# decisiongraph/leann-rs

Hardware: AMD Instinct MI355X
Metric: queries/sec @ recall@10>=0.95 (higher is better)
Workload: dtype f32

## Files before the change

### leann-rs_amd/csrc/search.cuh

```cuda
#pragma once
#include "common.cuh"
#include "row_screen.h"
#include "search_plan.h"

struct GraphView {
    const float *X;
    const uint32_t *adj0;
    const uint32_t *adjU;
    const uint32_t *upper_off;
    uint64_t n;
    uint32_t d, ld, M, M0, max_level, entry;
    uint32_t feat_h, row_bytes;
    const float *norms;
};

#define GPOOL_TABLES 1024u
#define GPOOL_BITS 16u

struct SearchArgs {
    const float *queries;
    const uint32_t *q_rows;
    uint32_t ldq, nq, k, ef, target_level;
    uint32_t hash_bits;
    uint64_t key_offset;
    uint64_t *out_keys;
    float *out_dists;
    uint32_t *out_counts;
    uint32_t *out_stats;
    uint64_t *out_expanded;
    uint32_t *out_nexp;
    uint32_t exp_cap;
    unsigned long long *gpool;
    uint32_t *gpool_lock;
    uint32_t *gpool_ctr;
    uint32_t gpool_bits, gpool_tables;
    unsigned long long *gpool2;
    uint32_t *gpool2_lock;
    uint32_t gpool2_bits, gpool2_tables;
    const uint8_t *allow;
    uint64_t allow_stride;
    const uint16_t *x_hi, *x_lo;
    uint32_t ldp;
    unsigned long long *screen_ctr;
};

static_assert(alignof(SearchArgs) == 8 && alignof(GraphView) == 8, "lazy_search_args assumes `a` sits at the 8-byte aligned offset behind `g`");
__device__ __forceinline__ const __attribute__((address_space(4))) SearchArgs *lazy_search_args() {
    typedef const __attribute__((address_space(4))) char *kptr;
    return (const __attribute__((address_space(4))) SearchArgs *)((kptr)__builtin_amdgcn_kernarg_segment_ptr() +
                                                                  ((sizeof(GraphView) + 7) & ~(size_t)7));
}

__device__ __forceinline__ uint32_t uni(uint32_t v) { return (uint32_t)__builtin_amdgcn_readfirstlane((int)v); }

__device__ __forceinline__ uint32_t vis_hash(uint32_t id, uint32_t bits) {
    return (id * 0x9E3779B1u) >> (32 - bits);
}

__device__ __forceinline__ bool vis_insert_lds(uint32_t *tab, uint32_t bits, uint32_t id) {
    const uint32_t mask = (1u << bits) - 1u;
    uint32_t h = vis_hash(id, bits);
    for (;;) {
        uint32_t old = atomicCAS(&tab[h], LEANN_EMPTY, id);
        if (old == LEANN_EMPTY) return true;
        if (old == id) return false;
        h = (h + 1) & mask;
    }
}
__device__ __forceinline__ bool vis_insert_hbm(unsigned long long *tab, uint32_t bits, uint32_t gen, uint32_t id) {
    const uint32_t mask = (1u << bits) - 1u;
    uint32_t h = vis_hash(id, bits);
    const unsigned long long mine = ((unsigned long long)gen << 32) | id;
    for (;;) {
        unsigned long long cur = __hip_atomic_load(&tab[h], __ATOMIC_RELAXED, __HIP_MEMORY_SCOPE_AGENT);
        if ((uint32_t)(cur >> 32) != gen) {
            unsigned long long prev = atomicCAS(&tab[h], cur, mine);
            if (prev == cur) return true;
            continue;
        }
        if ((uint32_t)cur == id) return false;
        h = (h + 1) & mask;
    }
}

template <int T, int R>
__device__ __forceinline__ void wave_dist_rows(const float4 (&q)[T], const float *__restrict__ X, uint32_t ld,
                                               const uint32_t (&ids)[R], int nrows, int lane, float (&out)[R]) {
    float4 v[R][T];
#pragma unroll
    for (int r = 0; r < R; r++) {
        if (r < nrows) {
            const float *row = X + (size_t)ids[r] * ld;
#pragma unroll
            for (int t = 0; t < T; t++) v[r][t] = row_load4(row, ld, t, lane);
        }
    }
#pragma unroll
    for (int r = 0; r < R; r++) {
        if (r < nrows) {
            float4 acc = make_float4(0.f, 0.f, 0.f, 0.f);
#pragma unroll
            for (int t = 0; t < T; t++) fma4(acc, q[t], v[r][t]);
            out[r] = 1.0f - wave_tree_sum(lane4_sum(acc));
        }
    }
}

__device__ __forceinline__ uint2 plane_tail_load(const uint16_t *__restrict__ row, uint32_t ldp, int c, int lane) {
    const uint32_t j = 256u * c + 4u * lane;
    return j < ldp ? *reinterpret_cast<const uint2 *>(row + j) : make_uint2(0u, 0u);
}
template <int T>
__device__ __forceinline__ void plane_row_load(const uint16_t *__restrict__ row, uint32_t ldp, int lane, uint2 (&h)[T]) {
#pragma unroll
    for (int p = 0; p < T / 2; p++) {
        if (512u * (uint32_t)(p + 1) <= ldp) {
            const uint4 v = *reinterpret_cast<const uint4 *>(row + 512 * p + 8 * lane);
            h[2 * p] = make_uint2(v.x, v.y);
            h[2 * p + 1] = make_uint2(v.z, v.w);
        } else {
            h[2 * p] = plane_tail_load(row, ldp, 2 * p, lane);
            h[2 * p + 1] = plane_tail_load(row, ldp, 2 * p + 1, lane);
        }
    }
    if (T & 1) h[T - 1] = plane_tail_load(row, ldp, T - 1, lane);
}
template <int T, int R>
__device__ __forceinline__ uint32_t wave_dist_rows_screen(const float4 (&q)[T], const uint16_t *__restrict__ Xhi, const uint16_t *__restrict__ Xlo,
                                                          uint32_t ldp, const uint32_t (&ids)[R], int nrows, int lane, bool armed, float worst,
                                                          float E, float (&out)[R]) {
    uint2 h[R][T], l[R][T];
#pragma unroll
    for (int r = 0; r < R; r++)
        if (r < nrows) plane_row_load<T>(Xhi + (size_t)ids[r] * ldp, ldp, lane, h[r]);
    uint32_t ruled = 0;
#pragma unroll
    for (int r = 0; r < R; r++) {
        if (r < nrows) {
            float4 s = make_float4(0.f, 0.f, 0.f, 0.f), a = make_float4(0.f, 0.f, 0.f, 0.f);
#pragma unroll
            for (int t = 0; t < T; t++) {
                float4 x;
                x.x = __uint_as_float(h[r][t].x << 16);
                x.y = __uint_as_float(h[r][t].x & 0xFFFF0000u);
                x.z = __uint_as_float(h[r][t].y << 16);
                x.w = __uint_as_float(h[r][t].y & 0xFFFF0000u);
                fma4(s, q[t], x);
                a.x = fmaf(fabsf(q[t].x), fabsf(x.x), a.x);
                a.y = fmaf(fabsf(q[t].y), fabsf(x.y), a.y);
                a.z = fmaf(fabsf(q[t].z), fabsf(x.z), a.z);
                a.w = fmaf(fabsf(q[t].w), fabsf(x.w), a.w);
            }
            const float lb = rs_lower_bound(wave_tree_sum(rs_lane_bound(lane4_sum(s), lane4_sum(a))), E);
            out[r] = lb;
            if (armed && lb > worst) ruled |= 1u << r;
        }
    }
#pragma unroll
    for (int r = 0; r < R; r++)
        if (r < nrows && !((ruled >> r) & 1u)) plane_row_load<T>(Xlo + (size_t)ids[r] * ldp, ldp, lane, l[r]);
#pragma unroll
    for (int r = 0; r < R; r++) {
        if (r < nrows && !((ruled >> r) & 1u)) {
            float4 acc = make_float4(0.f, 0.f, 0.f, 0.f);
#pragma unroll
            for (int t = 0; t < T; t++) {
                float4 x;
                x.x = __uint_as_float((h[r][t].x << 16) | (l[r][t].x & 0xFFFFu));
                x.y = __uint_as_float((h[r][t].x & 0xFFFF0000u) | (l[r][t].x >> 16));
                x.z = __uint_as_float((h[r][t].y << 16) | (l[r][t].y & 0xFFFFu));
                x.w = __uint_as_float((h[r][t].y & 0xFFFF0000u) | (l[r][t].y >> 16));
                fma4(acc, q[t], x);
            }
            out[r] = 1.0f - wave_tree_sum(lane4_sum(acc));
        }
    }
    return ruled;
}

template <int T, int R>
__device__ __forceinline__ void wave_dist_rows_feat(const float4 (&q)[T], const char *__restrict__ Xb, uint32_t row_bytes,
                                                    uint32_t h, const uint32_t (&ids)[R], int nrows, int lane, float (&out)[R],
                                                    const float *__restrict__ norms = nullptr) {
    uint2 v[R][T];
    float nrm[R];
#pragma unroll
    for (int r = 0; r < R; r++) {
        if (r < nrows) {
            const char *row = Xb + (size_t)ids[r] * row_bytes;
#pragma unroll
            for (int t = 0; t < T; t++) {
                const uint32_t j = 256u * t + 4u * lane;
                v[r][t] = j < h ? *reinterpret_cast<const uint2 *>(row + 2 * (size_t)j) : make_uint2(0u, 0u);
            }
            nrm[r] = norms ? norms[ids[r]] : *reinterpret_cast<const float *>(row + 2 * (size_t)h);
        }
    }
#pragma unroll
    for (int r = 0; r < R; r++) {
        if (r < nrows) {
            float4 acc = make_float4(0.f, 0.f, 0.f, 0.f);
#pragma unroll
            for (int t = 0; t < T; t++) {
                float4 x;
                x.x = __uint_as_float(v[r][t].x << 16);
                x.y = __uint_as_float(v[r][t].x & 0xFFFF0000u);
                x.z = __uint_as_float(v[r][t].y << 16);
                x.w = __uint_as_float(v[r][t].y & 0xFFFF0000u);
                fma4(acc, q[t], x);
            }
            out[r] = 1.0f - wave_tree_sum(lane4_sum(acc)) / nrm[r];
        }
    }
}

template <int T, int R>
__device__ __forceinline__ void wave_dist_rows_bf16(const float4 (&q)[T], const uint16_t *__restrict__ Xb, uint32_t ldb,
                                                    const uint32_t (&ids)[R], int nrows, int lane, float (&out)[R]) {
    uint2 v[R][T];
#pragma unroll
    for (int r = 0; r < R; r++)
        if (r < nrows) plane_row_load<T>(Xb + (size_t)ids[r] * ldb, ldb, lane, v[r]);
#pragma unroll
    for (int r = 0; r < R; r++) {
        if (r < nrows) {
            float4 acc = make_float4(0.f, 0.f, 0.f, 0.f);
#pragma unroll
            for (int t = 0; t < T; t++) {
                float4 x;
                x.x = __uint_as_float(v[r][t].x << 16);
                x.y = __uint_as_float(v[r][t].x & 0xFFFF0000u);
                x.z = __uint_as_float(v[r][t].y << 16);
                x.w = __uint_as_float(v[r][t].y & 0xFFFF0000u);
                fma4(acc, q[t], x);
            }
            out[r] = 1.0f - wave_tree_sum(lane4_sum(acc));
        }
    }
}

typedef uint32_t u32x4_a8 __attribute__((ext_vector_type(4), aligned(8)));
__device__ __forceinline__ float feat8_partial_pair(const float (&q)[8], const u32x4_a8 v) {
    float4 lo, hi;
    lo.x = fmaf(q[0], __uint_as_float(v.x << 16), 0.f);
    lo.y = fmaf(q[1], __uint_as_float(v.x & 0xFFFF0000u), 0.f);
    lo.z = fmaf(q[2], __uint_as_float(v.y << 16), 0.f);
    lo.w = fmaf(q[3], __uint_as_float(v.y & 0xFFFF0000u), 0.f);
    hi.x = fmaf(q[4], __uint_as_float(v.z << 16), 0.f);
    hi.y = fmaf(q[5], __uint_as_float(v.z & 0xFFFF0000u), 0.f);
    hi.z = fmaf(q[6], __uint_as_float(v.w << 16), 0.f);
    hi.w = fmaf(q[7], __uint_as_float(v.w & 0xFFFF0000u), 0.f);
    return lane4_sum(lo) + lane4_sum(hi);
}
template <int G>
__device__ __forceinline__ void group_dist_rows_feat256(const float (&qa)[8], const float (&qb)[8], const char *__restrict__ Xb,
                                                        uint32_t row_bytes, const uint32_t (&id)[G], const bool (&valid)[G], int lane,
                                                        float (&out)[G], const float *__restrict__ norms) {
    const int m = lane & 15;
    u32x4_a8 va[G], vb[G];
    float nrm[G];
#pragma unroll
    for (int g = 0; g < G; g++) {
        va[g] = vb[g] = u32x4_a8{0u, 0u, 0u, 0u};
        nrm[g] = 1.f;
        if (valid[g]) {
            const char *row = Xb + (size_t)id[g] * row_bytes;
            va[g] = *reinterpret_cast<const u32x4_a8 *>(row + 16 * m);
            vb[g] = *reinterpret_cast<const u32x4_a8 *>(row + 256 + 16 * m);
            if (m == 15) nrm[g] = norms ? norms[id[g]] : *reinterpret_cast<const float *>(row + 512);
        }
    }
#pragma unroll
    for (int g = 0; g < G; g++) {
        float sa = feat8_partial_pair(qa, va[g]), sb = feat8_partial_pair(qb, vb[g]);
        sa = dpp_pair_add<0xB1, 0xf>(sa);
        sb = dpp_pair_add<0xB1, 0xf>(sb);
        sa = dpp_pair_add<0x4E, 0xf>(sa);
        sb = dpp_pair_add<0x4E, 0xf>(sb);
        sa = dpp_pair_add<0x114, 0xf>(sa);
        sb = dpp_pair_add<0x114, 0xf>(sb);
        sa = dpp_pair_add<0x118, 0xf>(sa);
        sb = dpp_pair_add<0x118, 0xf>(sb);
        out[g] = 1.0f - (sa + sb) / nrm[g];
    }
}

__device__ __forceinline__ const uint32_t *adj_list(const uint32_t *__restrict__ base, const uint32_t *__restrict__ upper_off, uint32_t deg,
                                                    int lv, uint32_t node) {
    const size_t list = lv == 0 ? (size_t)node : (size_t)upper_off[node] + (uint32_t)(lv - 1);
    return base + list * deg;
}

struct SearchLds {
    uint64_t *s_key;
    uint32_t *s_new;
    uint32_t *misc;
};

template <int T, int R, int NW, bool FEAT, bool FILT = false, bool G16 = false, int LW = 1, bool SCREEN = false, bool BF16 = false>
__device__ void beam_search_one(const GraphView &g, const SearchArgs &a, uint32_t qi, unsigned char *smem) {
    const int tid = threadIdx.x, lane = tid & 63, wave = tid >> 6;
    const auto *const za = lazy_search_args();
    const uint32_t ef = a.ef;
    static_assert(LW == 1 || LW == 2, "lists of at most 128 ids");
    static_assert(!SCREEN || (NW == 4 && !FEAT && !FILT && !G16 && LW == 1), "the row screen exists in the plain throughput form only");
    static_assert(!BF16 || (!FEAT && !G16 && !SCREEN), "bf16 rows: stored vectors, whole rows");
    const uint32_t maxdeg = g.M0 > g.M ? g.M0 : g.M;
    const uint32_t efp = (ef + 1) & ~1u;
    SearchLds s;
    uint64_t *const W0 = reinterpret_cast<uint64_t *>(smem);
    constexpr uint32_t NBUF = NW > 4 ? 2u : 1u;
    const uint32_t kstride = maxdeg + 8;
    s.s_key = W0 + 2 * efp;
    s.s_new = reinterpret_cast<uint32_t *>(s.s_key + NBUF * kstride);
    s.misc = s.s_new + NBUF * maxdeg;
    size_t off = 2 * (size_t)efp * 8 + NBUF * ((size_t)maxdeg + 8) * 8 + NBUF * (size_t)maxdeg * 4 + 64;
    off = (off + 15) & ~(size_t)15;
    const uint32_t kf = FILT ? a.k : 0u, kfp = (kf + 1) & ~1u;
    uint64_t *const R0 = reinterpret_cast<uint64_t *>(smem + off);
    uint64_t *const s_keyR = R0 + 2 * kfp;
    const uint8_t *const allow = FILT ? a.allow + (size_t)qi * a.allow_stride : nullptr;
    uint32_t rsize = 0;
    int rcur = 0;
    if (FILT) off += 2 * (size_t)kfp * 8 + NBUF * ((size_t)maxdeg + 8) * 8;
    uint32_t *table = reinterpret_cast<uint32_t *>(smem + off);
    const uint32_t hbits = a.hash_bits, hsize = 1u << hbits;
    uint32_t vis_limit = hsize - (hsize >> 2);
    uint32_t hbm = 0;
    unsigned long long *gtab = nullptr;
    uint32_t gslot = 0, gen = 0, gbits = 0;

    float4 q[T];
    float qa[8], qb[8];
    {
        const float *qv;
        uint32_t dq = FEAT ? g.feat_h : g.d;
        if (!FEAT && a.q_rows) qv = g.X + (size_t)a.q_rows[qi] * g.ld;
        else qv = a.queries + (size_t)qi * a.ldq;
#pragma unroll
        for (int t = 0; t < T; t++)
            if (!G16) q[t] = vec_load4_guard(qv, dq, t, lane);
        if (G16) {
#pragma unroll
            for (int i = 0; i < 8; i++) {
                qa[i] = qv[8 * (lane & 15) + i];
                qb[i] = qv[128 + 8 * (lane & 15) + i];
            }
        }
    }

    float rs_E = 0.f;
    uint32_t rs_ruled = 0;
    if constexpr (SCREEN) {
        float4 qs = make_float4(0.f, 0.f, 0.f, 0.f);
#pragma unroll
        for (int t = 0; t < T; t++) { qs.x += fabsf(q[t].x); qs.y += fabsf(q[t].y); qs.z += fabsf(q[t].z); qs.w += fabsf(q[t].w); }
        rs_E = rs_abs_term(wave_tree_sum(lane4_sum(qs)));
        if (tid == 0) s.misc[10] = 0;
    }
    const uint32_t *const adj0_p = g.adj0, *const adjU_p = g.adjU, *const upoff_p = g.upper_off;
    uint32_t n_evals = 1, hops0 = 0, hopsU = 0;
    uint32_t n_vis = 0;
    uint64_t best;
    {
        uint32_t ids[1] = {g.entry};
        float dd[1];
        if (G16) {
            const bool valid[1] = {lane < 16};
            group_dist_rows_feat256<1>(qa, qb, reinterpret_cast<const char *>(g.X), g.row_bytes, ids, valid, lane, dd, g.norms);
            dd[0] = __int_as_float(__builtin_amdgcn_readlane(__float_as_int(dd[0]), 15));
        } else if (FEAT) wave_dist_rows_feat<T, 1>(q, reinterpret_cast<const char *>(g.X), g.row_bytes, g.feat_h, ids, 1, lane, dd, g.norms);
        else if constexpr (BF16) wave_dist_rows_bf16<T, 1>(q, reinterpret_cast<const uint16_t *>(g.X), g.row_bytes >> 1, ids, 1, lane, dd);
        else wave_dist_rows<T, 1>(q, g.X, g.ld, ids, 1, lane, dd);
        best = make_key(dd[0], g.entry);
    }

#ifdef LEANN_STAMPS
    uint64_t stamp[8] = {0, 0, 0, 0, 0, 0, 0, 0};
#endif
    uint32_t wsize = 0, level_hops = 0;
    int cur = 0;
    bool aborted = false;
    for (int lv = (int)g.max_level; lv >= (int)a.target_level; --lv) {
        const uint32_t ef_l = (lv == (int)a.target_level) ? ef : 1u;
        const uint32_t deg = lv == 0 ? g.M0 : g.M;
        if (!hbm)
            for (uint32_t i = tid; i < hsize; i += NW * 64) table[i] = LEANN_EMPTY;
        __syncthreads();
        if (tid == 0) {
            W0[0] = best;
            if (hbm) {
                gen = atomicAdd(&za->gpool_ctr[1], 1u) + 1u;
                s.misc[5] = gen;
                vis_insert_hbm(gtab, gbits, gen, key_id(best));
            } else {
                table[vis_hash(key_id(best), hbits)] = key_id(best);
            }
            s.misc[1] = LEANN_EMPTY;
            s.misc[2] = LEANN_EMPTY;
            s.misc[3] = 0;
            if (FILT && lv == (int)a.target_level) {
                const uint32_t e = key_id(best);
                const uint32_t ok = (allow[e >> 3] >> (e & 7)) & 1u;
                if (ok) R0[0] = best;
                s.misc[6] = ok;
            }
        }
        __syncthreads();
        if (hbm) gen = uni(s.misc[5]);
        const bool filt_level = FILT && lv == (int)a.target_level;
        if (filt_level) { rsize = uni(s.misc[6]); rcur = 0; }
        cur = 0;
        wsize = 1;
        n_vis = 1;
        uint32_t sel = 0;
        uint32_t hop = 0;
        constexpr bool EARLY_B = NW > 4;
        if constexpr (!EARLY_B) {
            uint32_t e_pref = LEANN_EMPTY, e_pref1 = LEANN_EMPTY;
            const uint32_t *const adj_base = lv == 0 ? adj0_p : adjU_p;
            if (wave == 0) {
                e_pref = (uint32_t)lane < deg ? adj_list(adj_base, upoff_p, deg, lv, key_id(best))[lane] : LEANN_EMPTY;
                if constexpr (LW == 2) e_pref1 = (uint32_t)lane + 64u < deg ? adj_list(adj_base, upoff_p, deg, lv, key_id(best))[lane + 64] : LEANN_EMPTY;
            }
            while (sel != LEANN_EMPTY) {
                uint64_t *Wc = W0 + cur * efp, *Wn = W0 + (cur ^ 1) * efp;
    #ifdef LEANN_STAMPS
                const uint64_t st0 = __builtin_amdgcn_s_memtime();
    #endif
                if (wave == 0) {
                    constexpr uint32_t p = 0;
                    const uint64_t ckey = Wc[sel];
                    const uint32_t hidx = hop;
                    #include "hop_adj.cuh"
                }
    #ifdef LEANN_STAMPS
                const uint64_t stB = __builtin_amdgcn_s_memtime();
    #endif
                __syncthreads();
    #ifdef LEANN_STAMPS
                const uint64_t stB1 = __builtin_amdgcn_s_memtime();
    #endif
                const uint32_t table_full = uni(s.misc[3]);
                if (table_full) {
                    #include "hop_migrate.cuh"
                    continue;
                }
                const uint32_t n_new = uni(s.misc[0]);
                uint64_t *const skey = s.s_key, *const skeyR = s_keyR;
                const uint32_t *const snew = s.s_new;
                if constexpr (SCREEN) {
                    const bool armed = wsize == ef_l;
                    const float worst = orderable_f32(uni((uint32_t)(Wc[wsize - 1] >> 32)));
                    for (uint32_t j0 = wave; j0 < n_new; j0 += NW * R) {
                        uint32_t ids[R];
                        float dd[R];
                        int nrows = 0;
    #pragma unroll
                        for (int r = 0; r < R; r++) {
                            uint32_t j = j0 + r * NW;
                            if (j < n_new) { ids[r] = s.s_new[j]; nrows = r + 1; }
                        }
                        const uint32_t ruled = wave_dist_rows_screen<T, R>(q, za->x_hi, za->x_lo, za->ldp, ids, nrows, lane, armed, worst, rs_E, dd);
                        rs_ruled += (uint32_t)__popc(ruled);
                        if (lane == 0) {
    #pragma unroll
                            for (int r = 0; r < R; r++)
                                if (r < nrows) s.s_key[j0 + r * NW] = make_key(dd[r], ids[r]);
                        }
                    }
                } else {
                    #include "hop_rows.cuh"
                }
    #ifdef LEANN_STAMPS
                const uint64_t stC = __builtin_amdgcn_s_memtime();
    #endif
                __syncthreads();
    #ifdef LEANN_STAMPS
                const uint64_t stB2 = __builtin_amdgcn_s_memtime();
    #endif
                uint32_t *next_slot = &s.misc[1 + (hop & 1)];
                const uint32_t n_pad = (n_new + 7) & ~7u;
                if (wave == 0) {
                    #include "hop_select.cuh"
                } else {
                    #include "hop_merge.cuh"
                }
                if (filt_level) {
                    #include "hop_rmerge.cuh"
                }
    #ifdef LEANN_STAMPS
                const uint64_t stD = __builtin_amdgcn_s_memtime();
    #endif
                __syncthreads();
    #ifdef LEANN_STAMPS
                {
                    const uint64_t stE = __builtin_amdgcn_s_memtime();
                    stamp[0] += stB - st0; stamp[1] += stB1 - stB; stamp[2] += stC - stB1; stamp[3] += stB2 - stC;
                    stamp[4] += stD - stB2; stamp[5] += stE - stD; stamp[6] += 1;
                }
    #endif
                sel = uni(*next_slot);
                wsize = min(wsize + n_new, ef_l);
                cur ^= 1;
                hop++;
            }
        } else {
            const uint32_t *const adj_base = lv == 0 ? adj0_p : adjU_p;
            uint32_t e_pref = LEANN_EMPTY, e_pref1 = LEANN_EMPTY;
            auto phase_b = [&](uint32_t p, uint64_t ckey, uint32_t hidx) __attribute__((always_inline)) {
                #include "hop_adj.cuh"
            };
            if (wave == 0) {
                e_pref = (uint32_t)lane < deg ? adj_list(adj_base, upoff_p, deg, lv, key_id(best))[lane] : LEANN_EMPTY;
                if constexpr (LW == 2) e_pref1 = (uint32_t)lane + 64u < deg ? adj_list(adj_base, upoff_p, deg, lv, key_id(best))[lane + 64] : LEANN_EMPTY;
                phase_b(0u, best, 0u);
            }
            __syncthreads();
            uint32_t par = 0;
            for (;;) {
                uint64_t *Wc = W0 + cur * efp, *Wn = W0 + (cur ^ 1) * efp;
#ifdef LEANN_STAMPS
                const uint64_t st0 = __builtin_amdgcn_s_memtime();
#endif
                if (uni(s.misc[3])) {
                    #include "hop_migrate.cuh"
                    if (wave == 0) phase_b(par, Wc[sel], hop);
                    __syncthreads();
                    continue;
                }
                const uint32_t n_new = uni(s.misc[8 + par]);
                uint64_t *const skey = s.s_key + par * kstride;
                const uint32_t *const snew = s.s_new + par * maxdeg;
                uint64_t *const skeyR = s_keyR + par * kstride;
                #include "hop_rows.cuh"
#ifdef LEANN_STAMPS
                const uint64_t stC = __builtin_amdgcn_s_memtime();
#endif
                __syncthreads();
#ifdef LEANN_STAMPS
                const uint64_t stB2 = __builtin_amdgcn_s_memtime();
#endif
                uint32_t *next_slot = &s.misc[1 + (hop & 1)];
                const uint32_t n_pad = (n_new + 7) & ~7u;
                if (wave == 0) {
                    #include "hop_select.cuh"
                    if (next != LEANN_EMPTY) phase_b(par ^ 1u, ckey, hop + 1);
                } else {
                    #include "hop_merge.cuh"
                }
                if (filt_level) {
                    #include "hop_rmerge.cuh"
                }
#ifdef LEANN_STAMPS
                const uint64_t stD = __builtin_amdgcn_s_memtime();
#endif
                __syncthreads();
#ifdef LEANN_STAMPS
                {
                    const uint64_t stE = __builtin_amdgcn_s_memtime();
                    stamp[0] += 0; stamp[1] += 0; stamp[2] += stC - st0; stamp[3] += stB2 - stC;
                    stamp[4] += stD - stB2; stamp[5] += stE - stD; stamp[6] += 1;
                }
#endif
                sel = uni(*next_slot);
                wsize = min(wsize + n_new, ef_l);
                cur ^= 1;
                hop++;
                par ^= 1u;
                if (sel == LEANN_EMPTY) break;
            }
        }
        level_hops = hop;
        if (aborted) break;
        best = W0[cur * efp] & ~1ull;
        __syncthreads();
    }

    __syncthreads();
    if (hbm && tid == 0) atomicExch(&(hbm == 1 ? za->gpool_lock : za->gpool2_lock)[gslot], 0u);
    if constexpr (SCREEN) {
        if (lane == 0 && rs_ruled) atomicAdd(&s.misc[10], rs_ruled);
        __syncthreads();
        if (tid == 0) {
            const uint32_t ruled = s.misc[10];
            atomicAdd(&za->screen_ctr[0], (unsigned long long)ruled);
            atomicAdd(&za->screen_ctr[1], (unsigned long long)(n_evals - 1u - ruled));
        }
    }
    if (aborted) {
        for (uint32_t t = tid; t < za->k; t += NW * 64) {
            za->out_keys[(size_t)qi * za->k + t] = 0xFFFFFFFFFFFFFFFFull;
            za->out_dists[(size_t)qi * za->k + t] = __uint_as_float(0x7F800000u);
        }
        if (tid == 0) {
            za->out_counts[qi] = 0;
            if (za->out_stats) {
                za->out_stats[(size_t)qi * 4 + 0] = n_evals;
                za->out_stats[(size_t)qi * 4 + 1] = hops0;
                za->out_stats[(size_t)qi * 4 + 2] = hopsU;
                za->out_stats[(size_t)qi * 4 + 3] = 3u;
            }
        }
        return;
    }
    const uint32_t nout = FILT ? rsize : min(wsize, za->k);
    uint64_t *Wc = FILT ? R0 + rcur * kfp : W0 + cur * efp;
    for (uint32_t t = tid; t < za->k; t += NW * 64) {
        size_t o = (size_t)qi * za->k + t;
        if (t < nout) {
            uint64_t k = Wc[t];
            za->out_keys[o] = (uint64_t)key_id(k) + za->key_offset;
            za->out_dists[o] = key_dist(k);
        } else {
            za->out_keys[o] = 0xFFFFFFFFFFFFFFFFull;
            za->out_dists[o] = __uint_as_float(0x7F800000u);
        }
    }
#ifdef LEANN_STAMPS
    if (tid == 0 && za->out_expanded == nullptr && za->exp_cap == 0xFEED) {
        unsigned long long *dst = reinterpret_cast<unsigned long long *>(za->out_nexp) + (size_t)qi * 8;
        for (int i = 0; i < 8; i++) dst[i] = stamp[i];
    }
#endif
    if (tid == 0) {
        za->out_counts[qi] = nout;
        if (za->out_nexp && za->exp_cap != 0xFEED) za->out_nexp[qi] = min(level_hops, za->exp_cap);
        if (za->out_stats) {
            za->out_stats[(size_t)qi * 4 + 0] = n_evals;
            za->out_stats[(size_t)qi * 4 + 1] = hops0;
            za->out_stats[(size_t)qi * 4 + 2] = hopsU;
            za->out_stats[(size_t)qi * 4 + 3] = hbm;
        }
    }
    __syncthreads();
}

#ifndef LEANN_T2_OCC
#define LEANN_T2_OCC 6
#endif
#ifndef LEANN_T1_OCC
#define LEANN_T1_OCC 8
#endif
template <int T, int R, int NW, bool BUILD>
__global__ void __launch_bounds__(NW * 64, (NW == 4 && T == 2) ? LEANN_T2_OCC : (NW == 4 && T == 1) ? LEANN_T1_OCC : 1) beam_search_kernel(GraphView g, SearchArgs a) {
    extern __shared__ __attribute__((aligned(16))) unsigned char smem[];
    uint32_t qi = blockIdx.x;
    if (qi >= a.nq) return;
    beam_search_one<T, R, NW, false>(g, a, qi, smem);
}
#ifndef LEANN_SCREEN_OCC3
#define LEANN_SCREEN_OCC3 4
#endif
#ifndef LEANN_SCREEN_OCC6
#define LEANN_SCREEN_OCC6 3
#endif
template <int T, int R>
__global__ void __launch_bounds__(256, T == 3 ? LEANN_SCREEN_OCC3 : LEANN_SCREEN_OCC6) beam_search_screen_kernel(GraphView g, SearchArgs a) {
    extern __shared__ __attribute__((aligned(16))) unsigned char smem[];
    uint32_t qi = blockIdx.x;
    if (qi >= a.nq) return;
    beam_search_one<T, R, 4, false, false, false, 1, true>(g, a, qi, smem);
}
template <int T, int R, int NW>
__global__ void __launch_bounds__(NW * 64) beam_search_filtered_kernel(GraphView g, SearchArgs a) {
    extern __shared__ __attribute__((aligned(16))) unsigned char smem[];
    uint32_t qi = blockIdx.x;
    if (qi >= a.nq) return;
    beam_search_one<T, R, NW, false, true>(g, a, qi, smem);
}
template <int T, int R, int NW>
__global__ void __launch_bounds__(NW * 64) beam_search_feat_filtered_kernel(GraphView g, SearchArgs a) {
    extern __shared__ __attribute__((aligned(16))) unsigned char smem[];
    uint32_t qi = blockIdx.x;
    if (qi >= a.nq) return;
    beam_search_one<T, R, NW, true, true>(g, a, qi, smem);
}
#ifndef LEANN_FEAT_OCC
#define LEANN_FEAT_OCC 8
#endif
#ifndef LEANN_FEAT256_OCC
#define LEANN_FEAT256_OCC 7
#endif
template <int G, int NW>
__global__ void __launch_bounds__(NW * 64, NW == 4 ? LEANN_FEAT256_OCC : 1) beam_search_feat256_kernel(GraphView g, SearchArgs a) {
    extern __shared__ __attribute__((aligned(16))) unsigned char smem[];
    uint32_t qi = blockIdx.x;
    if (qi >= a.nq) return;
    beam_search_one<1, G, NW, true, false, true>(g, a, qi, smem);
}
template <int G, int NW>
__global__ void __launch_bounds__(NW * 64) beam_search_feat256_filtered_kernel(GraphView g, SearchArgs a) {
    extern __shared__ __attribute__((aligned(16))) unsigned char smem[];
    uint32_t qi = blockIdx.x;
    if (qi >= a.nq) return;
    beam_search_one<1, G, NW, true, true, true>(g, a, qi, smem);
}
template <int T, int R, int NW>
__global__ void __launch_bounds__(NW * 64, (NW == 4 && T == 1) ? LEANN_FEAT_OCC : 1) beam_search_feat_kernel(GraphView g, SearchArgs a) {
    extern __shared__ __attribute__((aligned(16))) unsigned char smem[];
    uint32_t qi = blockIdx.x;
    if (qi >= a.nq) return;
    beam_search_one<T, R, NW, true>(g, a, qi, smem);
}

template <int T, int R, int NW, bool BUILD>
__global__ void __launch_bounds__(NW * 64) wide_beam_search_kernel(GraphView g, SearchArgs a) {
    extern __shared__ __attribute__((aligned(16))) unsigned char smem[];
    uint32_t qi = blockIdx.x;
    if (qi >= a.nq) return;
    beam_search_one<T, R, NW, false, false, false, 2>(g, a, qi, smem);
}
template <int T, int R, int NW>
__global__ void __launch_bounds__(NW * 64) wide_beam_search_filtered_kernel(GraphView g, SearchArgs a) {
    extern __shared__ __attribute__((aligned(16))) unsigned char smem[];
    uint32_t qi = blockIdx.x;
    if (qi >= a.nq) return;
    beam_search_one<T, R, NW, false, true, false, 2>(g, a, qi, smem);
}
template <int T, int R, int NW>
__global__ void __launch_bounds__(NW * 64) wide_beam_search_feat_kernel(GraphView g, SearchArgs a) {
    extern __shared__ __attribute__((aligned(16))) unsigned char smem[];
    uint32_t qi = blockIdx.x;
    if (qi >= a.nq) return;
    beam_search_one<T, R, NW, true, false, false, 2>(g, a, qi, smem);
}
template <int T, int R, int NW>
__global__ void __launch_bounds__(NW * 64) wide_beam_search_feat_filtered_kernel(GraphView g, SearchArgs a) {
    extern __shared__ __attribute__((aligned(16))) unsigned char smem[];
    uint32_t qi = blockIdx.x;
    if (qi >= a.nq) return;
    beam_search_one<T, R, NW, true, true, false, 2>(g, a, qi, smem);
}
template <int G, int NW>
__global__ void __launch_bounds__(NW * 64) wide_beam_search_feat256_kernel(GraphView g, SearchArgs a) {
    extern __shared__ __attribute__((aligned(16))) unsigned char smem[];
    uint32_t qi = blockIdx.x;
    if (qi >= a.nq) return;
    beam_search_one<1, G, NW, true, false, true, 2>(g, a, qi, smem);
}
template <int G, int NW>
__global__ void __launch_bounds__(NW * 64) wide_beam_search_feat256_filtered_kernel(GraphView g, SearchArgs a) {
    extern __shared__ __attribute__((aligned(16))) unsigned char smem[];
    uint32_t qi = blockIdx.x;
    if (qi >= a.nq) return;
    beam_search_one<1, G, NW, true, true, true, 2>(g, a, qi, smem);
}
```

Baseline: 1.298 million.

## Split screening into hi-plane bound pass then compact survivors for full distance

For T==3 the screened distance path now runs in two phases. First, H rows per wave load only the high bf16 plane and compute a lower bound used to rule rows out. Then only the survivors are compacted and their hi and lo planes loaded to compute exact distances, R rows at a time. The aim is to avoid loading the lo plane for rows that get ruled out, and to keep the wave busy on survivors rather than masked slots. The cost is more control flow and an extra pass over hi-plane data for rows that survive.

```diff
diff --git a/leann-rs_amd/csrc/search.cuh b/leann-rs_amd/csrc/search.cuh
--- a/leann-rs_amd/csrc/search.cuh
+++ b/leann-rs_amd/csrc/search.cuh
@@ -176,6 +176,86 @@
         }
     }
     return ruled;
+}
+
+#ifndef LEANN_SCREEN_H3
+#define LEANN_SCREEN_H3 7
+#endif
+template <int T, int H, int NW>
+__device__ __forceinline__ uint32_t wave_screen_hi_rows(const float4 (&q)[T], const uint16_t *__restrict__ Xhi, uint32_t ldp,
+                                                        const uint32_t *snew, uint64_t *skey, uint32_t j0, uint32_t n_new, int lane,
+                                                        float worst, float E) {
+    uint2 h[H][T];
+#pragma unroll
+    for (int r = 0; r < H; r++) {
+        if (j0 + r * NW < n_new) {
+            const uint32_t id = uni(snew[j0 + r * NW]);
+            plane_row_load<T>(Xhi + (size_t)id * ldp, ldp, lane, h[r]);
+        }
+    }
+    uint32_t surv = 0;
+#pragma unroll
+    for (int r = 0; r < H; r++) {
+        if (j0 + r * NW < n_new) {
+            float4 s = make_float4(0.f, 0.f, 0.f, 0.f), a = make_float4(0.f, 0.f, 0.f, 0.f);
+#pragma unroll
+            for (int t = 0; t < T; t++) {
+                float4 x;
+                x.x = __uint_as_float(h[r][t].x << 16);
+                x.y = __uint_as_float(h[r][t].x & 0xFFFF0000u);
+                x.z = __uint_as_float(h[r][t].y << 16);
+                x.w = __uint_as_float(h[r][t].y & 0xFFFF0000u);
+                fma4(s, q[t], x);
+                a.x = fmaf(fabsf(q[t].x), fabsf(x.x), a.x);
+                a.y = fmaf(fabsf(q[t].y), fabsf(x.y), a.y);
+                a.z = fmaf(fabsf(q[t].z), fabsf(x.z), a.z);
+                a.w = fmaf(fabsf(q[t].w), fabsf(x.w), a.w);
+            }
+            const float lb = rs_lower_bound(wave_tree_sum(rs_lane_bound(lane4_sum(s), lane4_sum(a))), E);
+            if (lb > worst) {
+                if (lane == 0) skey[j0 + r * NW] = make_key(lb, snew[j0 + r * NW]);
+            } else {
+                surv |= 1u << r;
+            }
+        }
+    }
+    return uni(surv);
+}
+template <int T, int R, int NW>
+__device__ __forceinline__ void wave_dist_rows_planes(const float4 (&q)[T], const uint16_t *__restrict__ Xhi, const uint16_t *__restrict__ Xlo,
+                                                      uint32_t ldp, const uint32_t *snew, uint64_t *skey, uint32_t j0, uint32_t surv, int lane) {
+    while (surv) {
+        uint2 h[R][T], l[R][T];
+        uint32_t m = surv;
+#pragma unroll
+        for (int r = 0; r < R; r++) {
+            if (m) {
+                const uint32_t id = uni(snew[j0 + (uint32_t)__builtin_ctz(m) * NW]);
+                m &= m - 1u;
+                plane_row_load<T>(Xhi + (size_t)id * ldp, ldp, lane, h[r]);
+                plane_row_load<T>(Xlo + (size_t)id * ldp, ldp, lane, l[r]);
+            }
+        }
+#pragma unroll
+        for (int r = 0; r < R; r++) {
+            if (surv) {
+                const uint32_t j = j0 + (uint32_t)__builtin_ctz(surv) * NW;
+                surv &= surv - 1u;
+                float4 acc = make_float4(0.f, 0.f, 0.f, 0.f);
+#pragma unroll
+                for (int t = 0; t < T; t++) {
+                    float4 x;
+                    x.x = __uint_as_float((h[r][t].x << 16) | (l[r][t].x & 0xFFFFu));
+                    x.y = __uint_as_float((h[r][t].x & 0xFFFF0000u) | (l[r][t].x >> 16));
+                    x.z = __uint_as_float((h[r][t].y << 16) | (l[r][t].y & 0xFFFFu));
+                    x.w = __uint_as_float((h[r][t].y & 0xFFFF0000u) | (l[r][t].y >> 16));
+                    fma4(acc, q[t], x);
+                }
+                const float dist = 1.0f - wave_tree_sum(lane4_sum(acc));
+                if (lane == 0) skey[j] = make_key(dist, snew[j]);
+            }
+        }
+    }
 }
 
 template <int T, int R>
@@ -452,6 +532,20 @@
                 if constexpr (SCREEN) {
                     const bool armed = wsize == ef_l;
                     const float worst = orderable_f32(uni((uint32_t)(Wc[wsize - 1] >> 32)));
+                    if constexpr (T == 3) {
+                        constexpr int H = LEANN_SCREEN_H3;
+                        static_assert(H >= 1 && H <= 16, "rows per wave in the hi round");
+                        const uint32_t w = uni((uint32_t)wave);
+                        for (uint32_t j0 = w; j0 < n_new; j0 += NW * H) {
+                            const uint32_t have = min((n_new - j0 + NW - 1) / NW, (uint32_t)H);
+                            uint32_t surv = (1u << have) - 1u;
+                            if (armed) {
+                                surv = wave_screen_hi_rows<T, H, NW>(q, za->x_hi, za->ldp, s.s_new, s.s_key, j0, n_new, lane, worst, rs_E);
+                                rs_ruled += have - (uint32_t)__popc(surv);
+                            }
+                            wave_dist_rows_planes<T, R, NW>(q, za->x_hi, za->x_lo, za->ldp, s.s_new, s.s_key, j0, surv, lane);
+                        }
+                    } else
                     for (uint32_t j0 = wave; j0 < n_new; j0 += NW * R) {
                         uint32_t ids[R];
                         float dd[R];
```

Result: faster. 1.407 million, median of 6 (+8.5%).
